# openai/procgen

Hardware: NVIDIA H100
Metric: env-steps/sec (higher is better)
Workload: dtype f32+u8

## Files before the change

### procgen_b200/csrc/pg_kernels.cuh

```cuda
#pragma once
#include "pg_raster.cuh"

namespace pg {

struct KParams {
    EnvHdr *hdr;
    Entity *ents;
    int16_t *grid;
    MT19937 *rng;
    MT19937 *lvl_rng;
    int32_t *scratch;
    RotBlit *rot_scratch;
    Blit *blit_list;
    unsigned char *frame_setup;
    Blit *cell_spill;
    const GameAssets *assets;
    const uint32_t *atlas;
    TileTable tiles;
    const int32_t *action;
    uint8_t *rgb;
    float *rew;
    uint8_t *first;
    int32_t *info_prev_level_seed;
    uint8_t *info_prev_level_complete;
    int32_t *info_level_seed;
    const uint32_t *lvl_seeds;
    int32_t *next_level_seed;
    int32_t ent_stride;
    int32_t grid_stride;
    int32_t scratch_stride;
    int32_t rot_stride;
    int32_t blit_stride;
    int32_t frame_setup_stride;
    int32_t cell_spill_stride;
    int32_t env_first, env_step, env_count;
    Options options;
    int32_t level_seed_low, level_seed_high;
    int32_t game_id;
    int32_t fixed_asset_seed;
    int32_t snap;
    int32_t env_global_offset;
    void *consumer;
    const uint16_t *consumer_lut;
    int32_t consumer_k;
    const int32_t *consumer_slot_dev;
    uint32_t *dbg_cycles;
    uint8_t *final_rgb;
    uint8_t *level_end;
    int32_t *reset_list;
    unsigned int *reset_count;
    const uint8_t *pause;
    uint8_t *paused;
    LevelBank bank;
    uint8_t *bank_level_end;
};

PG_HD Ctx make_ctx(const KParams &p, int env) {
    Ctx c;
    c.h = p.hdr + env;
    c.ents = p.ents + (size_t)env * p.ent_stride;
    c.grid = p.grid + (size_t)env * p.grid_stride;
    c.rng = p.rng + env;
    c.lvl_rng = p.lvl_rng + env;
    c.assets = p.assets;
    c.scratch = p.scratch + (size_t)env * p.scratch_stride;
    c.ent_cap = p.ent_stride - 1;
    c.grid_cap = p.grid_stride;
    c.scratch_cap = p.scratch_stride;
    c.obst_hi = -1;
    c.rot_scratch_raw = (p.rot_scratch && p.rot_stride > 0) ? (void *)(p.rot_scratch + (size_t)env * p.rot_stride) : nullptr;
    c.blit_list = p.blit_list ? p.blit_list + (size_t)env * p.blit_stride : nullptr;
    c.cell_spill = p.cell_spill ? p.cell_spill + (size_t)env * p.cell_spill_stride : nullptr;
    ctx_refresh(c);
    return c;
}

PG_HD void write_step_outputs(const KParams &p, int env, const EnvHdr &h) {
    p.rew[env] = h.reward;
    p.first[env] = (uint8_t)(h.done != 0);
    p.info_prev_level_seed[env] = h.prev_level_seed;
    p.info_prev_level_complete[env] = (uint8_t)(h.level_complete != 0);
    p.info_level_seed[env] = h.current_level_seed;
}

template <class G, class Frame>
PG_HD void env_init_logic(const KParams &p, int env) {
    Ctx c = make_ctx(p, env);
    G::init_constants(c);
    ctx_refresh(c);
    EnvHdr &h = *c.h;
    h.options = p.options;
    h.game_id = p.game_id;
    h.fixed_asset_seed = p.fixed_asset_seed;
    h.game_n = p.env_global_offset + env;
    h.level_seed_low = p.level_seed_low;
    h.level_seed_high = p.level_seed_high;
    mt_seed(*c.lvl_rng, p.lvl_seeds[env]);
    c.rng->seeded = 0;
    Engine<G>::reset(c);
    h.initial_reset_complete = 1;
    Raster<G, Frame>::prepare_camera(c);
    write_step_outputs(p, env, h);
}

#if defined(__CUDACC__)
__device__ __forceinline__ void pg_prefetch_line(const void *ptr) {
    asm volatile("prefetch.global.L1 [%0];" ::"l"(ptr));
}
__device__ __forceinline__ void env_prefetch(const KParams &p, int env) {
    const int lane = (int)(threadIdx.x & 31u);
    const char *hdr = reinterpret_cast<const char *>(p.hdr + env);
    if (lane < (int)((sizeof(EnvHdr) + 127) / 128))
        pg_prefetch_line(hdr + lane * 128);
    const MT19937 *rng = p.rng + env;
    if (lane == 8)
        pg_prefetch_line(&rng->p);
    const Entity *ents = p.ents + (size_t)env * p.ent_stride;
    const int n = p.hdr[env].n_ents;
    for (int i = lane; i < n; i += 32) pg_prefetch_line(ents + i);
    if (lane == 9) {
        int k = rng->p >= 624 ? 0 : rng->p;
        pg_prefetch_line(&rng->mt[k]);
        pg_prefetch_line(&rng->mt[(k + 397) % 624]);
    }
    if (lane >= 16 && lane < 24 && n > 0) {
        const EnvHdr &h = p.hdr[env];
        const Entity &a = ents[h.agent_idx];
        int row = (int)a.y + (lane - 16) - 3;
        if (row >= 0 && row < h.main_height) {
            int col = (int)a.x - 4;
            if (col < 0) col = 0;
            pg_prefetch_line(p.grid + (size_t)env * p.grid_stride + row * h.main_width + col);
        }
    }
    __syncwarp();
}
#endif

template <class G, class Frame, bool LEVEL_CHOICE = false>
PG_HD void env_step_logic(const KParams &p, int env) {
#if defined(__CUDA_ARCH__)
    env_prefetch(p, env);
#endif
    Ctx c = make_ctx(p, env);
    c.h->action = p.action[env];
    if (LEVEL_CHOICE) {
        const bool do_reset = Engine<G>::step_play(c);
        const int32_t next_seed = do_reset ? p.next_level_seed[env] : -1;
        if (Engine<G>::step_finish(c, do_reset, next_seed))
            p.next_level_seed[env] = -1;
    } else {
        Engine<G>::step(c);
    }
    Raster<G, Frame>::prepare_camera(c);
    write_step_outputs(p, env, *c.h);
}

template <bool FINAL>
PG_HD bool env_pause_logic(const KParams &p, int env) {
    const uint8_t paused = p.pause[env] != 0;
    p.paused[env] = paused;
    if (paused) {
        p.rew[env] = 0.f;
        p.first[env] = 0;
        if (FINAL)
            p.level_end[env] = 0;
    }
    return paused != 0;
}

template <class G, class Frame>
PG_HD bool env_step_logic_final(const KParams &p, int env) {
#if defined(__CUDA_ARCH__)
    env_prefetch(p, env);
#endif
    Ctx c = make_ctx(p, env);
    c.h->action = p.action[env];
    uint8_t cause = 0;
    const bool do_reset = Engine<G>::template step_play<true>(c, &cause);
    p.level_end[env] = cause;
    if (!do_reset)
        Engine<G>::step_finish(c, false, -1);
    Raster<G, Frame>::prepare_camera(c);
    if (!do_reset)
        write_step_outputs(p, env, *c.h);
    return do_reset;
}

template <class G, class Frame, bool BANK = false>
PG_HD void env_finish_logic(const KParams &p, int env) {
    Ctx c = make_ctx(p, env);
    const int32_t next_seed = p.next_level_seed ? p.next_level_seed[env] : -1;
    if (Engine<G>::template step_finish<BANK>(c, true, next_seed, &p.bank))
        p.next_level_seed[env] = -1;
    Raster<G, Frame>::prepare_camera(c);
    write_step_outputs(p, env, *c.h);
}

PG_HD size_t bank_stage_bytes(const KParams &p) {
    return sizeof(EnvHdr) + (size_t)p.ent_stride * sizeof(Entity) + (((size_t)p.grid_stride * sizeof(int16_t) + 15) & ~(size_t)15) +
           sizeof(MT19937) + (((size_t)p.scratch_stride * sizeof(int32_t) + 15) & ~(size_t)15);
}

template <class G>
PG_HD void bank_generate_level(const KParams &p, int item, unsigned char *stage) {
    const LevelBank &b = p.bank;
    Ctx c;
    c.h = reinterpret_cast<EnvHdr *>(stage);
    c.ents = reinterpret_cast<Entity *>(stage + sizeof(EnvHdr));
    c.grid = reinterpret_cast<int16_t *>(stage + sizeof(EnvHdr) + (size_t)p.ent_stride * sizeof(Entity));
    c.rng = reinterpret_cast<MT19937 *>(reinterpret_cast<unsigned char *>(c.grid) + (((size_t)p.grid_stride * sizeof(int16_t) + 15) & ~(size_t)15));
    c.scratch = reinterpret_cast<int32_t *>(c.rng + 1);
    c.lvl_rng = nullptr;
    c.assets = p.assets;
    c.ent_cap = p.ent_stride - 1;
    c.grid_cap = p.grid_stride;
    c.scratch_cap = p.scratch_stride;
    c.obst_hi = -1;
    c.rot_scratch_raw = nullptr;
    c.blit_list = nullptr;
    c.cell_spill = nullptr;
    G::init_constants(c);
    EnvHdr &h = *c.h;
    h.options = p.options;
    h.options.center_agent = BANK_CENTER_AGENT_UNSET;
    h.game_id = p.game_id;
    h.fixed_asset_seed = p.fixed_asset_seed;
    h.level_seed_low = p.level_seed_low;
    h.level_seed_high = p.level_seed_high;
    h.current_level_seed = b.seeds[item];
    h.episodes_remaining = 1;
    ctx_refresh(c);
    mt_seed(*c.rng, (uint32_t)h.current_level_seed);
    G::game_reset(c);
    unsigned char *slot = b.slots + (size_t)item * b.slot_bytes;
    const bool usable = h.max_ents_seen <= G::ENT_CAP && h.grid_size <= G::GRID_CAP && h.agent_idx < c.ent_cap;
    if (usable) {
        bank_copy_vecs(slot + BANK_SLOT_HEAD, &h, (int)sizeof(EnvHdr));
        bank_copy_vecs(slot + b.ents_off, c.ents, h.n_ents * (int)sizeof(Entity));
        int16_t *dg = reinterpret_cast<int16_t *>(slot + b.grid_off);
        const int16_t *sg = c.grid;
        pg_warp_for(h.grid_size, [=](int k) { dg[k] = sg[k]; });
        bank_copy_vecs(slot + b.rng_off, c.rng, (int)sizeof(MT19937));
        int32_t *ds = reinterpret_cast<int32_t *>(slot + b.scratch_off);
        const int32_t *ss = c.scratch + G::PERSIST_SCRATCH_FIRST;
        pg_warp_for(G::PERSIST_SCRATCH_WORDS, [=](int k) { ds[k] = ss[k]; });
    }
    *reinterpret_cast<int32_t *>(slot) = usable ? 1 : 0;
}

template <class G, class Setup>
PG_HD void env_setup_frame(const KParams &p, int env, Setup &f, int lane, int nlanes) {
    Ctx c = make_ctx(p, env);
    using R = Raster<G, Setup>;
    R::setup_frame(c, f, p.snap != 0, lane, nlanes);
#if defined(__CUDA_ARCH__)
    __syncwarp();
#endif
    R::build_entity_blits(c, f, lane, nlanes);
#if defined(__CUDA_ARCH__)
    __syncwarp();
#endif
    if (f.n_jobs > 0) {
        R::frame_tiles(c, f, lane, nlanes);
#if defined(__CUDA_ARCH__)
        __syncwarp();
#endif
    }
    if (G::DEFER_ROTATED) {
        R::frame_rots(c, f, lane, nlanes);
#if defined(__CUDA_ARCH__)
        __syncwarp();
#endif
    }
    if (lane == 0)
        R::frame_append_overlays(f);
    if (G::DRAWS_GRID) {
#if defined(__CUDA_ARCH__)
        __syncwarp();
#endif
        R::frame_build(c, f, lane, nlanes, 0);
#if defined(__CUDA_ARCH__)
        __syncwarp();
#endif
        R::frame_tile_alloc(c, f, p.tiles, lane, nlanes);
#if defined(__CUDA_ARCH__)
        __syncwarp();
#endif
        R::frame_cells_finish(c, f, lane, nlanes);
    } else {
        R::frame_build(c, f, lane, nlanes, 0);
    }
}

template <class Frame>
PG_HD void env_stage_tiles_serial(const KParams &p, Frame &f) {
    const int nj = f.n_tjobs < MAX_TILE_JOBS ? f.n_tjobs : MAX_TILE_JOBS;
    for (int j = 0; j < nj; j++)
        for (int w = 0; w < (int)f.tjob_words[j]; w++) f.arena[f.tjob_dst[j] + w] = p.tiles.texels[f.tjob_src[j] + w];
}

template <class G, class Frame>
PG_HD void env_render_compose(const KParams &p, Frame &f, int row_first, int row_step, int lane, int nlanes) {
    Raster<G, Frame>::compose_rows(f, f.fb, row_first, row_step, lane, nlanes, p.atlas);
}

PG_HD void tile_table_fill(const SpriteDesc *sprites, const uint32_t *index, uint32_t *texels, const uint32_t *atlas, int slot, int tw, int th, int tid,
                           int nthreads) {
    Blit b;
    make_image_blit(b, 0.0, 0.0, (double)tw, (double)th, sprites[slot], false, 256, true);
    uint32_t *dst = texels + index[(slot * MAX_TILE_DIM + (tw - 1)) * MAX_TILE_DIM + (th - 1)];
    const int words = tile_words(tw, th);
    for (int i = tid; i < words; i += nthreads) {
        const int dy = i / tw, dx = i - dy * tw;
        dst[i] = dy < th ? tile_texel(b, atlas, dx, dy) : 0u;
    }
}

template <class G, int VIEW = G::MAX_VIEW_CELLS>
struct FrameFor {
    using type = FrameT<(G::DRAWS_GRID ? VIEW : 1), G::MAX_VISIBLE_ENTS, G::MAX_ROT_BLITS>;
    using setup = FrameSetupT<(G::DRAWS_GRID ? VIEW : 1), G::MAX_VISIBLE_ENTS, G::MAX_ROT_BLITS>;
    using shared = typename type::Shared;
};

}
```

### procgen_b200/csrc/pg_launch.cuh

```cuda
#pragma once
#include <stdarg.h>
#include <stdio.h>
#include <stdlib.h>
#include <string.h>

#include "pg_kernels.cuh"

#ifndef PG_HOSTSIM
#include <cuda_runtime.h>
#endif

namespace pg {

static inline void pg_fatal(const char *fmt, ...) {
    fprintf(stderr, "fatal: ");
    va_list args;
    va_start(args, fmt);
    vfprintf(stderr, fmt, args);
    va_end(args);
    exit(EXIT_FAILURE);
}
#define pg_fassert(cond)                                                                  \
    do {                                                                                  \
        if (!(cond)) {                                                                    \
            fprintf(stderr, "fassert failed '%s' at %s:%d\n", #cond, __FILE__, __LINE__); \
            exit(EXIT_FAILURE);                                                           \
        }                                                                                 \
    } while (0)

#ifndef PG_HOSTSIM
#define CUDA_CHECK(expr)                                                                          \
    do {                                                                                          \
        cudaError_t _e = (expr);                                                                  \
        if (_e != cudaSuccess)                                                                    \
            pg_fatal("CUDA error %s at %s:%d: %s\n", cudaGetErrorName(_e), __FILE__, __LINE__, cudaGetErrorString(_e)); \
    } while (0)
#endif

#ifndef PG_LOGIC_WARPS
#define PG_LOGIC_WARPS 2
#endif
#ifndef PG_LOGIC_MIN_BLOCKS
#define PG_LOGIC_MIN_BLOCKS 24
#endif
#ifndef PG_STEP_CHUNKS
#define PG_STEP_CHUNKS 8
#endif
#ifndef PG_AUX_STREAMS
#define PG_AUX_STREAMS 16
#endif
constexpr int kLogicThreads = 32 * PG_LOGIC_WARPS;
constexpr int kLogicEnvsPerBlock = PG_LOGIC_WARPS;
constexpr int kRenderThreads = 128;

#ifndef PG_HOSTSIM
template <class G, bool INIT, bool LEVEL_CHOICE = false, bool FINAL = false, bool PAUSE = false>
__global__ void __launch_bounds__(kLogicThreads, PG_LOGIC_MIN_BLOCKS) logic_kernel(KParams p, unsigned int *ticket) {
    using Frame = typename FrameFor<G>::type;
    const unsigned lane = threadIdx.x & 31u;
    while (true) {
        unsigned t = 0;
        if (lane == 0)
            t = atomicAdd(ticket, 1u);
        t = __shfl_sync(0xffffffffu, t, 0);
        if (t >= (unsigned)p.env_count)
            break;
        const int env = p.env_first + (int)t * p.env_step;
        const long long t0 = p.dbg_cycles ? clock64() : 0;
        if (INIT)
            env_init_logic<G, Frame>(p, env);
        else if (PAUSE && env_pause_logic<FINAL>(p, env)) {
        } else if (FINAL) {
            if (env_step_logic_final<G, Frame>(p, env) && lane == 0)
                p.reset_list[atomicAdd(p.reset_count, 1u)] = env;
        } else
            env_step_logic<G, Frame, LEVEL_CHOICE>(p, env);
        __syncwarp();
        if (p.dbg_cycles && lane == 0)
            p.dbg_cycles[env] = (uint32_t)(clock64() - t0);
    }
}

template <class G, bool BANK = false>
__global__ void __launch_bounds__(kLogicThreads, PG_LOGIC_MIN_BLOCKS) finish_kernel(KParams p, unsigned int *ticket) {
    using Frame = typename FrameFor<G>::type;
    const unsigned lane = threadIdx.x & 31u;
    const unsigned count = *p.reset_count;
    while (true) {
        unsigned t = 0;
        if (lane == 0)
            t = atomicAdd(ticket, 1u);
        t = __shfl_sync(0xffffffffu, t, 0);
        if (t >= count)
            break;
        const int env = p.reset_list[t];
        const long long t0 = (BANK && p.dbg_cycles) ? clock64() : 0;
        env_finish_logic<G, Frame, BANK>(p, env);
        __syncwarp();
        if (BANK && p.dbg_cycles && lane == 0)
            p.dbg_cycles[env] += (uint32_t)(clock64() - t0);
    }
}

template <class G>
__global__ void __launch_bounds__(kLogicThreads) bank_build_kernel(KParams p, unsigned char *stage, int count, int warps) {
    const int w = (int)((blockIdx.x * blockDim.x + threadIdx.x) >> 5);
    if (w >= warps)
        return;
    for (int item = w; item < count; item += warps) {
        bank_generate_level<G>(p, item, stage + (size_t)w * bank_stage_bytes(p));
        __syncwarp();
    }
}

constexpr int kSetupThreads = 128;
#ifndef PG_SETUP_MIN_BLOCKS
#define PG_SETUP_MIN_BLOCKS 8
#endif
template <class G, int VIEW, bool LIST = false, bool PAUSE = false>
__global__ void __launch_bounds__(kSetupThreads, PG_SETUP_MIN_BLOCKS) setup_kernel(KParams p) {
    using Setup = typename FrameFor<G, VIEW>::setup;
    const int i = (int)blockIdx.x * (kSetupThreads / 32) + (int)(threadIdx.x >> 5);
    if (LIST) {
        const int count = (int)*p.reset_count;
        for (int j = i; j < count; j += (int)gridDim.x * (kSetupThreads / 32)) {
            const int env = p.reset_list[j];
            Setup &f = *reinterpret_cast<Setup *>(p.frame_setup + (size_t)env * p.frame_setup_stride);
            env_setup_frame<G, Setup>(p, env, f, (int)(threadIdx.x & 31u), 32);
        }
        return;
    }
    if (i >= p.env_count)
        return;
    const int env = p.env_first + i * p.env_step;
    if (PAUSE && p.paused[env])
        return;
    Setup &f = *reinterpret_cast<Setup *>(p.frame_setup + (size_t)env * p.frame_setup_stride);
    env_setup_frame<G, Setup>(p, env, f, (int)(threadIdx.x & 31u), 32);
}

#ifndef PG_RENDER_CTAS_PER_SM
#define PG_RENDER_CTAS_PER_SM 0
#endif
template <class G, int VIEW>
struct RenderTune {
    static constexpr size_t kFrameBytes = sizeof(typename FrameFor<G, VIEW>::type);
#ifdef PG_RENDER_MIN_BLOCKS
    static constexpr int kMinBlocks = PG_RENDER_MIN_BLOCKS;
#else
    static constexpr int kFit = (int)((227 * 1024) / (kFrameBytes + 1024 + 16));
    static constexpr int kWant = G::DRAWS_GRID ? 7 : 8;
    static constexpr int kMinBlocks = kFit >= kWant ? kWant : (kFit >= 1 ? kFit : 1);
#endif
};

__device__ __forceinline__ uint32_t pg_smem_addr(const void *ptr) { return (uint32_t)__cvta_generic_to_shared(ptr); }
__device__ __forceinline__ void pg_mbar_init(unsigned long long *bar, unsigned count) {
    asm volatile("mbarrier.init.shared::cta.b64 [%0], %1;" ::"r"(pg_smem_addr(bar)), "r"(count) : "memory");
    asm volatile("fence.mbarrier_init.release.cluster;" ::: "memory");
}
__device__ __forceinline__ void pg_mbar_arrive_expect_tx(unsigned long long *bar, unsigned bytes) {
    asm volatile("mbarrier.arrive.expect_tx.shared::cta.b64 _, [%0], %1;" ::"r"(pg_smem_addr(bar)), "r"(bytes) : "memory");
}
__device__ __forceinline__ void pg_mbar_wait(unsigned long long *bar, unsigned parity) {
    unsigned done = 0;
    while (!done) {
        asm volatile(
            "{\n"
            ".reg .pred p;\n"
            "mbarrier.try_wait.parity.shared::cta.b64 p, [%1], %2;\n"
            "selp.u32 %0, 1, 0, p;\n"
            "}\n"
            : "=r"(done)
            : "r"(pg_smem_addr(bar)), "r"(parity)
            : "memory");
    }
}
__device__ __forceinline__ void pg_bulk_load(void *dst_smem, const void *src_gmem, unsigned bytes, unsigned long long *bar) {
    asm volatile("cp.async.bulk.shared::cluster.global.mbarrier::complete_tx::bytes [%0], [%1], %2, [%3];" ::"r"(pg_smem_addr(dst_smem)),
                 "l"(src_gmem), "r"(bytes), "r"(pg_smem_addr(bar))
                 : "memory");
}
__device__ __forceinline__ void pg_bulk_store_and_wait(void *dst_gmem, const void *src_smem, unsigned bytes) {
    asm volatile("cp.async.bulk.global.shared::cta.bulk_group [%0], [%1], %2;" ::"l"(dst_gmem), "r"(pg_smem_addr(src_smem)), "r"(bytes) : "memory");
    asm volatile("cp.async.bulk.commit_group;" ::: "memory");
    asm volatile("cp.async.bulk.wait_group.read 0;" ::: "memory");
}

template <class G, int VIEW, int PASS, class EnvOf>
__device__ __forceinline__ void render_env_frame(const KParams &p, typename FrameFor<G, VIEW>::type &f, EnvOf env_of, unsigned parity) {
    using Frame = typename FrameFor<G, VIEW>::type;
    const int tid = (int)threadIdx.x;
#ifdef PG_PHASE_TIMING
    long long t0 = clock64(), t1;
#define PG_RENDER_PHASE(id)                                       \
    do {                                                          \
        t1 = clock64();                                           \
        if (tid == 0)                                             \
            p.hdr[env_of()].dbg_phase[id] = (uint32_t)(t1 - t0);       \
        t0 = t1;                                                  \
    } while (0)
#else
#define PG_RENDER_PHASE(id) do { } while (0)
#endif
    using Shared = typename FrameFor<G, VIEW>::shared;
    using Setup = typename FrameFor<G, VIEW>::setup;
    const Setup *gs = reinterpret_cast<const Setup *>(p.frame_setup + (size_t)env_of() * p.frame_setup_stride);
    if (tid < 32) {
        const int nj = G::DRAWS_GRID ? (gs->n_tjobs < MAX_TILE_JOBS ? gs->n_tjobs : MAX_TILE_JOBS) : 0;
        unsigned words = 0;
        for (int j = tid; j < nj; j += 32) words += gs->tjob_words[j];
        for (int d = 16; d > 0; d >>= 1) words += __shfl_xor_sync(0xffffffffu, words, d);
        if (tid == 0) {
            pg_mbar_arrive_expect_tx(&f.mbar, (unsigned)sizeof(Shared) + 4u * words);
            pg_bulk_load(static_cast<Shared *>(&f), static_cast<const Shared *>(gs), (unsigned)sizeof(Shared), &f.mbar);
        }
        __syncwarp();
        for (int j = tid; j < nj; j += 32)
            pg_bulk_load(f.arena + gs->tjob_dst[j], p.tiles.texels + gs->tjob_src[j], 4u * gs->tjob_words[j], &f.mbar);
    }
    pg_mbar_wait(&f.mbar, parity);
    PG_RENDER_PHASE(0);
    env_render_compose<G, Frame>(p, f, tid >> 5, kRenderThreads >> 5, tid & 31, 32);
    __syncthreads();
    PG_RENDER_PHASE(5);
    if (p.consumer != nullptr && !(PASS == 1 && p.level_end[env_of()] != 0)) {
        const int kf = p.consumer_k, s = *p.consumer_slot_dev;
        const int slots = kf == 1 ? 1 : 2 * kf;
        uint32_t *base = reinterpret_cast<uint32_t *>(p.consumer) + (size_t)env_of() * slots * (3 * RES_W * RES_H / 2);
        const uint16_t *lut = p.consumer_lut;
        for (int pair = tid; pair < RES_W * RES_H / 2; pair += kRenderThreads) {
            const uint32_t c0 = f.fb[2 * pair], c1 = f.fb[2 * pair + 1];
#pragma unroll
            for (int ch = 0; ch < 3; ch++) {
                const int sh = 16 - 8 * ch;
                const uint32_t v = (uint32_t)lut[(c0 >> sh) & 0xffu] | ((uint32_t)lut[(c1 >> sh) & 0xffu] << 16);
                base[(size_t)(s * 3 + ch) * (RES_W * RES_H / 2) + pair] = v;
                if (kf > 1)
                    base[(size_t)((s + kf) * 3 + ch) * (RES_W * RES_H / 2) + pair] = v;
            }
        }
        if (kf > 1 && p.first[env_of()]) {
            for (int j = 1; j < kf; j++) {
                const int a = (s + j) % kf;
                for (int w = tid; w < 3 * RES_W * RES_H / 2; w += kRenderThreads) {
                    base[(size_t)a * (3 * RES_W * RES_H / 2) + w] = 0u;
                    base[(size_t)(a + kf) * (3 * RES_W * RES_H / 2) + w] = 0u;
                }
            }
        }
    }
    {
        constexpr int kQuadsPerThread = RES_W * RES_H / 4 / kRenderThreads;
        uint32_t c[kQuadsPerThread][4];
#pragma unroll
        for (int j = 0; j < kQuadsPerThread; j++) {
            const uint4 v = reinterpret_cast<const uint4 *>(f.fb)[tid + j * kRenderThreads];
            c[j][0] = v.x; c[j][1] = v.y; c[j][2] = v.z; c[j][3] = v.w;
        }
        __syncthreads();
#pragma unroll
        for (int j = 0; j < kQuadsPerThread; j++) Raster<G, Frame>::pack_quad(c[j], f.fb + 3 * (tid + j * kRenderThreads));
    }
    asm volatile("fence.proxy.async.shared::cta;" ::: "memory");
    __syncthreads();
    PG_RENDER_PHASE(6);
    if (tid == 0)
        pg_bulk_store_and_wait((PASS == 1 && p.level_end[env_of()] != 0 ? p.final_rgb : p.rgb) + (size_t)env_of() * (RES_W * RES_H * 3), f.fb,
                               RES_W * RES_H * 3);
    PG_RENDER_PHASE(7);
#undef PG_RENDER_PHASE
}

__device__ __forceinline__ void consumer_repeat_frame(const KParams &p, int env) {
    constexpr int kSlotVecs = 3 * RES_W * RES_H * 2 / 16;
    const int kf = p.consumer_k, s = *p.consumer_slot_dev;
    uint4 *base = reinterpret_cast<uint4 *>(p.consumer) + (size_t)env * (2 * kf) * kSlotVecs;
    const uint4 *src = base + (size_t)((s - 1 + kf) % kf) * kSlotVecs;
    for (int w = (int)threadIdx.x; w < kSlotVecs; w += kRenderThreads) {
        const uint4 v = src[w];
        base[(size_t)s * kSlotVecs + w] = v;
        base[(size_t)(s + kf) * kSlotVecs + w] = v;
    }
}

template <class G, int VIEW, int PASS = 0, bool PAUSE = false>
__global__ void __launch_bounds__(kRenderThreads, RenderTune<G, VIEW>::kMinBlocks) render_kernel(KParams p) {
    static_assert(!(PAUSE && PASS == 2), "phase B's list never holds a paused env");
    using Frame = typename FrameFor<G, VIEW>::type;
    extern __shared__ __align__(128) unsigned char smem_raw[];
    Frame &f = *reinterpret_cast<Frame *>(smem_raw);
    if (PAUSE && p.paused[p.env_first + (int)blockIdx.x * p.env_step]) {
        if (p.consumer != nullptr && p.consumer_k > 1)
            consumer_repeat_frame(p, p.env_first + (int)blockIdx.x * p.env_step);
        return;
    }
    if (threadIdx.x == 0)
        pg_mbar_init(&f.mbar, 1);
    __syncthreads();
    if (PASS == 2) {
        __shared__ int list_env;
        for (unsigned i = 0;; i++) {
            const int j = (int)(blockIdx.x + i * gridDim.x);
            if (j >= (int)*p.reset_count)
                break;
            if (threadIdx.x == 0)
                list_env = p.reset_list[j];
            __syncthreads();
            render_env_frame<G, VIEW, PASS>(p, f, [&] { return list_env; }, i & 1u);
            __syncthreads();
        }
        return;
    }
    render_env_frame<G, VIEW, PASS>(p, f, [&] { return p.env_first + (int)blockIdx.x * p.env_step; }, 0);
}

#endif

#ifndef PG_HOSTSIM
template <class G>
__global__ void camera_kernel(KParams p) {
    using Frame = typename FrameFor<G>::type;
    if (threadIdx.x == 0 && blockIdx.x < (unsigned)p.env_count) {
        const int env = p.env_first + (int)blockIdx.x * p.env_step;
        Ctx c = make_ctx(p, env);
        Raster<G, Frame>::prepare_camera(c);
        write_step_outputs(p, env, *c.h);
    }
}
#endif

template <class G, int VIEW, int PASS>
void render_env_serial(const KParams &p, int env) {
    using Frame = typename FrameFor<G, VIEW>::type;
    using Setup = typename FrameFor<G, VIEW>::setup;
    using Shared = typename FrameFor<G, VIEW>::shared;
    static thread_local Frame *f = new Frame;
    Setup &s = *reinterpret_cast<Setup *>(p.frame_setup + (size_t)env * p.frame_setup_stride);
    env_setup_frame<G, Setup>(p, env, s, 0, 1);
    static_cast<Shared &>(*f) = static_cast<const Shared &>(s);
    env_stage_tiles_serial<Frame>(p, *f);
    for (int w = 0; w < 4; w++) env_render_compose<G, Frame>(p, *f, w, 4, 0, 1);
    uint8_t *rgb = PASS == 1 && p.level_end[env] != 0 ? p.final_rgb : p.rgb;
    uint32_t *out = reinterpret_cast<uint32_t *>(rgb + (size_t)env * (RES_W * RES_H * 3));
    for (int g = 0; g < RES_W * RES_H / 4; g++) Raster<G, Frame>::pack_quad(f->fb + 4 * g, out + 3 * g);
}

struct LaunchCtx {
#ifndef PG_HOSTSIM
    cudaStream_t stream;
    cudaStream_t logic_stream;
    cudaEvent_t link;
    int max_logic_blocks;
    int num_sms;
    int render_smem_floor;
    cudaEvent_t *tev;
#endif
    unsigned int *ticket;
    int64_t *launch_counter;
};

#ifndef PG_HOSTSIM
template <class G, int VIEW, int PASS = 0, bool PAUSE = false>
int prepare_render_smem(const LaunchCtx &lc) {
    using Frame = typename FrameFor<G, VIEW>::type;
    const int bytes = (int)sizeof(Frame) > lc.render_smem_floor ? (int)sizeof(Frame) : lc.render_smem_floor;
    static int attr_set[64] = {};
    int dev = 0;
    CUDA_CHECK(cudaGetDevice(&dev));
    int &have = attr_set[dev & 63];
    if (have < bytes) {
        CUDA_CHECK(cudaFuncSetAttribute(render_kernel<G, VIEW, PASS, PAUSE>, cudaFuncAttributeMaxDynamicSharedMemorySize, bytes));
        have = bytes;
    }
    return bytes;
}

static inline int logic_grid(const KParams &p, const LaunchCtx &lc) {
    const int blocks = (p.env_count + kLogicEnvsPerBlock - 1) / kLogicEnvsPerBlock;
    return blocks < lc.max_logic_blocks ? blocks : lc.max_logic_blocks;
}
#endif


template <class G, bool INIT, bool LEVEL_CHOICE, bool FINAL, bool PAUSE>
void logic_phase(const KParams &p, const LaunchCtx &lc) {
    constexpr size_t kTicketBytes = (FINAL ? 3 : 1) * sizeof(unsigned int);
#ifndef PG_HOSTSIM
    const cudaStream_t ls = !FINAL && lc.logic_stream ? lc.logic_stream : lc.stream;
    CUDA_CHECK(cudaMemsetAsync(lc.ticket, 0, kTicketBytes, ls));
    if (lc.tev)
        CUDA_CHECK(cudaEventRecord(lc.tev[0], ls));
    logic_kernel<G, INIT, LEVEL_CHOICE, FINAL, PAUSE><<<logic_grid(p, lc), kLogicThreads, 0, ls>>>(p, lc.ticket);
    CUDA_CHECK(cudaGetLastError());
    if (ls != lc.stream) {
        CUDA_CHECK(cudaEventRecord(lc.link, ls));
        CUDA_CHECK(cudaStreamWaitEvent(lc.stream, lc.link, 0));
    }
#else
    using Frame = typename FrameFor<G>::type;
    memset(lc.ticket, 0, kTicketBytes);
    for (int i = 0; i < p.env_count; i++) {
        const int env = p.env_first + i * p.env_step;
        if (INIT)
            env_init_logic<G, Frame>(p, env);
        else if (PAUSE && env_pause_logic<FINAL>(p, env)) {
        } else if (FINAL) {
            if (env_step_logic_final<G, Frame>(p, env))
                p.reset_list[(*p.reset_count)++] = env;
        } else
            env_step_logic<G, Frame, LEVEL_CHOICE>(p, env);
    }
#endif
}

template <class G, bool BANK>
void finish_phase(const KParams &p, const LaunchCtx &lc) {
#ifndef PG_HOSTSIM
    finish_kernel<G, BANK><<<logic_grid(p, lc), kLogicThreads, 0, lc.stream>>>(p, lc.ticket + 2);
    CUDA_CHECK(cudaGetLastError());
#else
    (void)lc;
    using Frame = typename FrameFor<G>::type;
    for (unsigned int j = 0; j < *p.reset_count; j++) env_finish_logic<G, Frame, BANK>(p, p.reset_list[j]);
#endif
}

template <class G, int VIEW, int PASS, bool PAUSE>
void frames_phase(const KParams &p, const LaunchCtx &lc) {
    constexpr bool LIST = PASS == 2;
#ifndef PG_HOSTSIM
    const int render_smem = prepare_render_smem<G, VIEW, PASS, PAUSE>(lc);
    int setup_blocks = (p.env_count + kSetupThreads / 32 - 1) / (kSetupThreads / 32);
    int render_blocks = p.env_count;
    if (LIST) {
        const int setup_fit = lc.num_sms * PG_SETUP_MIN_BLOCKS, render_fit = lc.num_sms * RenderTune<G, VIEW>::kMinBlocks;
        setup_blocks = setup_blocks < setup_fit ? setup_blocks : setup_fit;
        render_blocks = render_blocks < render_fit ? render_blocks : render_fit;
    }
    if (lc.tev)
        CUDA_CHECK(cudaEventRecord(lc.tev[1], lc.stream));
    setup_kernel<G, VIEW, LIST, PAUSE><<<setup_blocks, kSetupThreads, 0, lc.stream>>>(p);
    if (lc.tev)
        CUDA_CHECK(cudaEventRecord(lc.tev[2], lc.stream));
    render_kernel<G, VIEW, PASS, PAUSE><<<render_blocks, kRenderThreads, render_smem, lc.stream>>>(p);
    if (lc.tev)
        CUDA_CHECK(cudaEventRecord(lc.tev[3], lc.stream));
    CUDA_CHECK(cudaGetLastError());
#else
    (void)lc;
    if (LIST) {
        for (unsigned int j = 0; j < *p.reset_count; j++) render_env_serial<G, VIEW, PASS>(p, p.reset_list[j]);
        return;
    }
    for (int i = 0; i < p.env_count; i++) {
        const int env = p.env_first + i * p.env_step;
        if (!(PAUSE && p.paused[env]))
            render_env_serial<G, VIEW, PASS>(p, env);
    }
#endif
}

template <class G, int VIEW, bool INIT, bool PAUSE, bool FINAL, bool BANK>
void launch_step(const KParams &p, const LaunchCtx &lc) {
    KParams q = p;
    q.reset_count = lc.ticket + 1;
    if constexpr (BANK && !FINAL)
        q.level_end = p.bank_level_end;
    if constexpr (FINAL || BANK)
        logic_phase<G, false, false, true, PAUSE>(q, lc);
    else if (!INIT && p.next_level_seed)
        logic_phase<G, false, true, false, PAUSE>(p, lc);
    else
        logic_phase<G, INIT, false, false, PAUSE>(p, lc);
    if constexpr (FINAL) {
        frames_phase<G, VIEW, 1, PAUSE>(q, lc);
        finish_phase<G, BANK>(q, lc);
        frames_phase<G, VIEW, 2, false>(q, lc);
    } else {
        if constexpr (BANK)
            finish_phase<G, true>(q, lc);
        frames_phase<G, VIEW, 0, PAUSE>(p, lc);
    }
    (*lc.launch_counter) += FINAL ? 6 : BANK ? 4 : 3;
}

template <class G, bool INIT, int VIEW>
void launch_env_kernel(const KParams &p, const LaunchCtx &lc) {
    if (p.env_count <= 0)
        return;
    if constexpr (INIT) {
        launch_step<G, VIEW, true, false, false, false>(p, lc);
        return;
    }
    switch ((p.pause ? 1 : 0) | (p.level_end ? 2 : 0) | (p.bank.slots ? 4 : 0)) {
    case 0: launch_step<G, VIEW, false, false, false, false>(p, lc); break;
    case 1: launch_step<G, VIEW, false, true, false, false>(p, lc); break;
    case 2: launch_step<G, VIEW, false, false, true, false>(p, lc); break;
    case 3: launch_step<G, VIEW, false, true, true, false>(p, lc); break;
    case 4: launch_step<G, VIEW, false, false, false, true>(p, lc); break;
    case 5: launch_step<G, VIEW, false, true, false, true>(p, lc); break;
    case 6: launch_step<G, VIEW, false, false, true, true>(p, lc); break;
    case 7: launch_step<G, VIEW, false, true, true, true>(p, lc); break;
    }
}

template <class G, int VIEW>
void launch_observe_only(const KParams &p, const LaunchCtx &lc) {
    if (p.env_count <= 0)
        return;
#ifndef PG_HOSTSIM
    camera_kernel<G><<<p.env_count, 32, 0, lc.stream>>>(p);
    CUDA_CHECK(cudaGetLastError());
#else
    using Frame = typename FrameFor<G>::type;
    for (int b = 0; b < p.env_count; b++) {
        int env = p.env_first + b * p.env_step;
        Ctx c = make_ctx(p, env);
        Raster<G, Frame>::prepare_camera(c);
        write_step_outputs(p, env, *c.h);
    }
#endif
    frames_phase<G, VIEW, 0, false>(p, lc);
    (*lc.launch_counter) += 2;
}

template <class G>
void launch_bank_build(const KParams &p, const LaunchCtx &lc, unsigned char *stage, int warps, int count) {
    if (count <= 0)
        return;
#ifndef PG_HOSTSIM
    const int blocks = (warps + kLogicEnvsPerBlock - 1) / kLogicEnvsPerBlock;
    bank_build_kernel<G><<<blocks, kLogicThreads, 0, lc.stream>>>(p, stage, count, warps);
    CUDA_CHECK(cudaGetLastError());
    (*lc.launch_counter) += 1;
#else
    (void)lc;
    (void)warps;
    for (int item = 0; item < count; item++) bank_generate_level<G>(p, item, stage);
#endif
}

struct GameVTable {
    const char *name;
    int id;
    int ent_cap, grid_cap, scratch_words;
    int rot_records;
    int blit_records;
    int setup_bytes[2];
    int cell_records[2];
    int frame_bytes[2];
    int render_ctas_per_sm[2];
    void (*init[2])(const KParams &, const LaunchCtx &);
    void (*step[2])(const KParams &, const LaunchCtx &);
    void (*observe_only[2])(const KParams &, const LaunchCtx &);
    void (*bank_build)(const KParams &, const LaunchCtx &, unsigned char *, int, int);
    int persist_scratch_words;
};

template <class G, int VIEW>
void fill_view(GameVTable &vt, int slot) {
    using F = FrameFor<G, VIEW>;
    vt.setup_bytes[slot] = (int)sizeof(typename F::setup);
    vt.cell_records[slot] = F::type::kMaxCells1D * F::type::kMaxCells1D;
    vt.frame_bytes[slot] = (int)sizeof(typename F::type);
#ifndef PG_HOSTSIM
    vt.render_ctas_per_sm[slot] = RenderTune<G, VIEW>::kMinBlocks;
#else
    vt.render_ctas_per_sm[slot] = 0;
#endif
    vt.init[slot] = &launch_env_kernel<G, true, VIEW>;
    vt.step[slot] = &launch_env_kernel<G, false, VIEW>;
    vt.observe_only[slot] = &launch_observe_only<G, VIEW>;
}

template <class G>
GameVTable make_vtable(int id) {
    GameVTable vt{};
    vt.name = G::NAME;
    vt.id = id;
    vt.ent_cap = G::ENT_CAP;
    vt.grid_cap = G::GRID_CAP;
    vt.scratch_words = G::SCRATCH_WORDS;
    vt.persist_scratch_words = G::PERSIST_SCRATCH_WORDS;
    vt.bank_build = &launch_bank_build<G>;
    vt.rot_records = FrameFor<G>::type::kMaxRot;
    vt.blit_records = FrameFor<G>::type::kMaxList;
    fill_view<G, G::MAX_VIEW_CELLS>(vt, 0);
    if constexpr (G::FULL_VIEW_CELLS > G::MAX_VIEW_CELLS)
        fill_view<G, G::FULL_VIEW_CELLS>(vt, 1);
    return vt;
}

}
```

Measured before the change: 20.43 million.

## Build setup frame in shared memory and store only the shared record to global

The setup kernel now builds each env's Setup struct in dynamic shared memory, one slot per warp, instead of working directly on the global per-env buffer. Once setup finishes, only the Shared portion is copied out with 16-byte vector stores, and the per-env global stride shrinks to sizeof(Shared). This is meant to cut global memory traffic from the many scattered writes and reads during setup. The cost is that setup occupancy may drop if the Setup struct is large, since launch bounds are now derived from how many blocks fit in shared memory. Optional clock64 phase timing instrumentation is also added.

```diff
diff --git a/procgen_b200/csrc/pg_kernels.cuh b/procgen_b200/csrc/pg_kernels.cuh
--- a/procgen_b200/csrc/pg_kernels.cuh
+++ b/procgen_b200/csrc/pg_kernels.cuh
@@ -249,14 +249,30 @@
     *reinterpret_cast<int32_t *>(slot) = usable ? 1 : 0;
 }
 
+#if defined(PG_PHASE_TIMING) && defined(__CUDA_ARCH__)
+#define PG_SETUP_PHASE_BEGIN long long _pg_s0 = clock64()
+#define PG_SETUP_PHASE(id)                                    \
+    do {                                                      \
+        const long long _pg_s1 = clock64();                   \
+        if (lane == 0)                                        \
+            p.hdr[env].dbg_phase[id] = (uint32_t)(_pg_s1 - _pg_s0); \
+        _pg_s0 = _pg_s1;                                      \
+    } while (0)
+#else
+#define PG_SETUP_PHASE_BEGIN do { } while (0)
+#define PG_SETUP_PHASE(id) do { } while (0)
+#endif
+
 template <class G, class Setup>
 PG_HD void env_setup_frame(const KParams &p, int env, Setup &f, int lane, int nlanes) {
+    PG_SETUP_PHASE_BEGIN;
     Ctx c = make_ctx(p, env);
     using R = Raster<G, Setup>;
     R::setup_frame(c, f, p.snap != 0, lane, nlanes);
 #if defined(__CUDA_ARCH__)
     __syncwarp();
 #endif
+    PG_SETUP_PHASE(1);
     R::build_entity_blits(c, f, lane, nlanes);
 #if defined(__CUDA_ARCH__)
     __syncwarp();
@@ -279,18 +295,33 @@
 #if defined(__CUDA_ARCH__)
         __syncwarp();
 #endif
+        PG_SETUP_PHASE(2);
         R::frame_build(c, f, lane, nlanes, 0);
 #if defined(__CUDA_ARCH__)
         __syncwarp();
 #endif
+        PG_SETUP_PHASE(3);
         R::frame_tile_alloc(c, f, p.tiles, lane, nlanes);
 #if defined(__CUDA_ARCH__)
         __syncwarp();
 #endif
+        PG_SETUP_PHASE(4);
         R::frame_cells_finish(c, f, lane, nlanes);
+        PG_SETUP_PHASE(8);
     } else {
+        PG_SETUP_PHASE(2);
         R::frame_build(c, f, lane, nlanes, 0);
-    }
+        PG_SETUP_PHASE(3);
+        PG_SETUP_PHASE(4);
+        PG_SETUP_PHASE(8);
+    }
+}
+
+template <class Setup>
+PG_HD void env_store_frame(const KParams &p, int env, const Setup &f) {
+    using Shared = typename Setup::Shared;
+    static_assert(sizeof(Shared) % 16 == 0, "the record is stored in 16-byte vectors");
+    bank_copy_vecs(p.frame_setup + (size_t)env * p.frame_setup_stride, static_cast<const Shared *>(&f), (int)sizeof(Shared));
 }
 
 template <class Frame>
diff --git a/procgen_b200/csrc/pg_launch.cuh b/procgen_b200/csrc/pg_launch.cuh
--- a/procgen_b200/csrc/pg_launch.cuh
+++ b/procgen_b200/csrc/pg_launch.cuh
@@ -117,16 +117,28 @@
 #ifndef PG_SETUP_MIN_BLOCKS
 #define PG_SETUP_MIN_BLOCKS 8
 #endif
+template <class G, int VIEW>
+struct SetupTune {
+    static constexpr int kSmemBytes = (int)sizeof(typename FrameFor<G, VIEW>::setup) * (kSetupThreads / 32);
+    static constexpr int kFit = (227 * 1024) / (kSmemBytes + 1024 + 128);
+    static constexpr int kMinBlocks = kFit >= PG_SETUP_MIN_BLOCKS ? PG_SETUP_MIN_BLOCKS : (kFit >= 1 ? kFit : 1);
+};
 template <class G, int VIEW, bool LIST = false, bool PAUSE = false>
-__global__ void __launch_bounds__(kSetupThreads, PG_SETUP_MIN_BLOCKS) setup_kernel(KParams p) {
+__global__ void __launch_bounds__(kSetupThreads, SetupTune<G, VIEW>::kMinBlocks) setup_kernel(KParams p) {
     using Setup = typename FrameFor<G, VIEW>::setup;
+    extern __shared__ __align__(128) unsigned char smem_raw[];
+    Setup &f = reinterpret_cast<Setup *>(smem_raw)[threadIdx.x >> 5];
+    const int lane = (int)(threadIdx.x & 31u);
     const int i = (int)blockIdx.x * (kSetupThreads / 32) + (int)(threadIdx.x >> 5);
     if (LIST) {
         const int count = (int)*p.reset_count;
         for (int j = i; j < count; j += (int)gridDim.x * (kSetupThreads / 32)) {
             const int env = p.reset_list[j];
-            Setup &f = *reinterpret_cast<Setup *>(p.frame_setup + (size_t)env * p.frame_setup_stride);
-            env_setup_frame<G, Setup>(p, env, f, (int)(threadIdx.x & 31u), 32);
+            env_setup_frame<G, Setup>(p, env, f, lane, 32);
+            __syncwarp();
+            PG_SETUP_PHASE_BEGIN;
+            env_store_frame<Setup>(p, env, f);
+            PG_SETUP_PHASE(9);
         }
         return;
     }
@@ -135,8 +147,11 @@
     const int env = p.env_first + i * p.env_step;
     if (PAUSE && p.paused[env])
         return;
-    Setup &f = *reinterpret_cast<Setup *>(p.frame_setup + (size_t)env * p.frame_setup_stride);
-    env_setup_frame<G, Setup>(p, env, f, (int)(threadIdx.x & 31u), 32);
+    env_setup_frame<G, Setup>(p, env, f, lane, 32);
+    __syncwarp();
+    PG_SETUP_PHASE_BEGIN;
+    env_store_frame<Setup>(p, env, f);
+    PG_SETUP_PHASE(9);
 }
 
 #ifndef PG_RENDER_CTAS_PER_SM
@@ -204,8 +219,7 @@
 #define PG_RENDER_PHASE(id) do { } while (0)
 #endif
     using Shared = typename FrameFor<G, VIEW>::shared;
-    using Setup = typename FrameFor<G, VIEW>::setup;
-    const Setup *gs = reinterpret_cast<const Setup *>(p.frame_setup + (size_t)env_of() * p.frame_setup_stride);
+    const Shared *gs = reinterpret_cast<const Shared *>(p.frame_setup + (size_t)env_of() * p.frame_setup_stride);
     if (tid < 32) {
         const int nj = G::DRAWS_GRID ? (gs->n_tjobs < MAX_TILE_JOBS ? gs->n_tjobs : MAX_TILE_JOBS) : 0;
         unsigned words = 0;
@@ -213,7 +227,7 @@
         for (int d = 16; d > 0; d >>= 1) words += __shfl_xor_sync(0xffffffffu, words, d);
         if (tid == 0) {
             pg_mbar_arrive_expect_tx(&f.mbar, (unsigned)sizeof(Shared) + 4u * words);
-            pg_bulk_load(static_cast<Shared *>(&f), static_cast<const Shared *>(gs), (unsigned)sizeof(Shared), &f.mbar);
+            pg_bulk_load(static_cast<Shared *>(&f), gs, (unsigned)sizeof(Shared), &f.mbar);
         }
         __syncwarp();
         for (int j = tid; j < nj; j += 32)
@@ -336,9 +350,11 @@
     using Setup = typename FrameFor<G, VIEW>::setup;
     using Shared = typename FrameFor<G, VIEW>::shared;
     static thread_local Frame *f = new Frame;
-    Setup &s = *reinterpret_cast<Setup *>(p.frame_setup + (size_t)env * p.frame_setup_stride);
-    env_setup_frame<G, Setup>(p, env, s, 0, 1);
-    static_cast<Shared &>(*f) = static_cast<const Shared &>(s);
+    static thread_local Setup *s = new Setup;
+    memset(static_cast<void *>(s), 0xA5, sizeof(Setup));
+    env_setup_frame<G, Setup>(p, env, *s, 0, 1);
+    env_store_frame<Setup>(p, env, *s);
+    static_cast<Shared &>(*f) = *reinterpret_cast<const Shared *>(p.frame_setup + (size_t)env * p.frame_setup_stride);
     env_stage_tiles_serial<Frame>(p, *f);
     for (int w = 0; w < 4; w++) env_render_compose<G, Frame>(p, *f, w, 4, 0, 1);
     uint8_t *rgb = PASS == 1 && p.level_end[env] != 0 ? p.final_rgb : p.rgb;
@@ -372,6 +388,19 @@
     if (have < bytes) {
         CUDA_CHECK(cudaFuncSetAttribute(render_kernel<G, VIEW, PASS, PAUSE>, cudaFuncAttributeMaxDynamicSharedMemorySize, bytes));
         have = bytes;
+    }
+    return bytes;
+}
+
+template <class G, int VIEW, bool LIST, bool PAUSE>
+int prepare_setup_smem() {
+    constexpr int bytes = SetupTune<G, VIEW>::kSmemBytes;
+    static bool attr_set[64] = {};
+    int dev = 0;
+    CUDA_CHECK(cudaGetDevice(&dev));
+    if (!attr_set[dev & 63]) {
+        CUDA_CHECK(cudaFuncSetAttribute(setup_kernel<G, VIEW, LIST, PAUSE>, cudaFuncAttributeMaxDynamicSharedMemorySize, bytes));
+        attr_set[dev & 63] = true;
     }
     return bytes;
 }
@@ -430,17 +459,18 @@
 void frames_phase(const KParams &p, const LaunchCtx &lc) {
     constexpr bool LIST = PASS == 2;
 #ifndef PG_HOSTSIM
+    const int setup_smem = prepare_setup_smem<G, VIEW, LIST, PAUSE>();
     const int render_smem = prepare_render_smem<G, VIEW, PASS, PAUSE>(lc);
     int setup_blocks = (p.env_count + kSetupThreads / 32 - 1) / (kSetupThreads / 32);
     int render_blocks = p.env_count;
     if (LIST) {
-        const int setup_fit = lc.num_sms * PG_SETUP_MIN_BLOCKS, render_fit = lc.num_sms * RenderTune<G, VIEW>::kMinBlocks;
+        const int setup_fit = lc.num_sms * SetupTune<G, VIEW>::kMinBlocks, render_fit = lc.num_sms * RenderTune<G, VIEW>::kMinBlocks;
         setup_blocks = setup_blocks < setup_fit ? setup_blocks : setup_fit;
         render_blocks = render_blocks < render_fit ? render_blocks : render_fit;
     }
     if (lc.tev)
         CUDA_CHECK(cudaEventRecord(lc.tev[1], lc.stream));
-    setup_kernel<G, VIEW, LIST, PAUSE><<<setup_blocks, kSetupThreads, 0, lc.stream>>>(p);
+    setup_kernel<G, VIEW, LIST, PAUSE><<<setup_blocks, kSetupThreads, setup_smem, lc.stream>>>(p);
     if (lc.tev)
         CUDA_CHECK(cudaEventRecord(lc.tev[2], lc.stream));
     render_kernel<G, VIEW, PASS, PAUSE><<<render_blocks, kRenderThreads, render_smem, lc.stream>>>(p);
@@ -561,7 +591,7 @@
 template <class G, int VIEW>
 void fill_view(GameVTable &vt, int slot) {
     using F = FrameFor<G, VIEW>;
-    vt.setup_bytes[slot] = (int)sizeof(typename F::setup);
+    vt.setup_bytes[slot] = (int)sizeof(typename F::shared);
     vt.cell_records[slot] = F::type::kMaxCells1D * F::type::kMaxCells1D;
     vt.frame_bytes[slot] = (int)sizeof(typename F::type);
 #ifndef PG_HOSTSIM
```

New measurement: 22.06 million, median of 6. 7.9% higher.
